# ThorLL/Element-Crush-Gym

Measured on AMD Instinct MI355X. Metric: env-steps/sec (batched boards) at 1/2/4/8 MI355X, 9×9×6; bit-exact vs CPU, higher is better.
Workload: dtype int8; 1 GPU; C3: 1,048,576 boards per GPU, 9x9x6, Match3Env.step x 7466 (step kernel + overflow fixup + autoreset; N>1: RCCL reward/done all-gather once after the last step); boards_per_gpu=1048576, num_moves=20, env_goal=500, parallelism=dp1, hw_queues=8, autoreset=True

## Files before the change

element-crush-gym_amd/csrc/m3_rules.hpp:

```cpp
#pragma once

#include <type_traits>

#include "m3_bitboard.hpp"
#include "m3_rng.hpp"

namespace m3 {

enum : int { PH_LOAD, PH_SWAP, PH_MATCH, PH_CLEAR, PH_DROP, PH_REFILL, PH_LEGAL, PH_NEXT, PH_RESET, PH_QUEUE,
             PH_STORE, PH_TBYTES, PH_TLOAD, PH_TATOM, PH_N };
template <class S, class = void>
struct HasProf : std::false_type {};
template <class S>
struct HasProf<S, std::void_t<decltype(S::PROF)>> : std::true_type {};
template <int K, class S>
M3_HD void mark(S& st) {
    if constexpr (HasProf<S>::value) st.template mark<K>();
}

constexpr int ceil_log2(int v) {
    int b = 0;
    while ((1 << b) < v) ++b;
    return b;
}

enum : uint32_t {
    FLAG_TERMINAL = 0x01u,
    FLAG_BAD_ACTION = 0x02u,
    FLAG_SHUFFLE_CAP = 0x04u,
    FLAG_NO_LEGAL = 0x08u,
    FLAG_SHUFFLED = 0x10u,
    FLAG_RNG_OVERFLOW = 0x20u,
    FLAG_GROUP_OVERFLOW = 0x40u,
    FLAG_RECOMPUTE = FLAG_RNG_OVERFLOW | FLAG_GROUP_OVERFLOW,
    FLAG_CASCADE_CAP = 0x100u,
    FLAG_RESET_CAP = 0x200u,
};
constexpr int CASCADE_CAP = 1 << 16;
template <class R, class = void>
struct DrawBounded : std::false_type {};
template <class R>
struct DrawBounded<R, std::void_t<decltype(R::DRAW_BOUNDED)>> : std::bool_constant<R::DRAW_BOUNDED> {};

template <class CF>
struct StaticDim;
template <class CF>
struct FrameDim;

template <int R_, int C_, int T_>
struct Cfg {
    static constexpr bool DYN = false;
    static constexpr int R = R_, C = C_, T = T_;
    static constexpr int N = R * C;
    static constexpr int W = (N + 31) / 32;
    static constexpr int BITS = ceil_log2(T + 1);
    static constexpr int TM = (1 << BITS) - 1;
    static constexpr int STM = (1 << (BITS + 1)) + 1 + TM;
    static constexpr int H = TM + 1;
    static constexpr int V = 2 * H;
    static constexpr int B = STM;
    static constexpr int M = TM + STM + 1;
    static constexpr int A = R * (C - 1) * 2;
    static constexpr int AW = (A + 31) / 32;
    static constexpr int NP = 7;
    static constexpr int MAXG = N / 3 + 1;
    static constexpr int SHUFFLE_CAP = 1024;
    static constexpr uint32_t TILE_RNG = (uint32_t)(T - 1);
    static constexpr uint32_t TILE_MASK = (1u << ceil_log2(T)) - 1u;
    static_assert(R >= 4 && C >= 4 && R <= 16 && C <= 16, "board size");
    static_assert(T >= 2 && BITS <= 4, "tile types must fit 4 bits");
    using Bd = BB<W>;
    using G = Geo<R, C, W>;
    using Dim = StaticDim<Cfg>;
};

template <int BITS_, int FS_ = 16>
struct FCfg {
    static constexpr bool DYN = true;
    static constexpr int FS = FS_;
    static_assert(FS == 16 || FS == 32, "frame side");
    static constexpr int R = FS, C = FS;
    static constexpr int N = R * C;
    static constexpr int W = N / 32;
    static constexpr int BITS = BITS_;
    static constexpr int TM = (1 << BITS) - 1;
    static constexpr int STM = (1 << (BITS + 1)) + 1 + TM;
    static constexpr int H = TM + 1;
    static constexpr int V = 2 * H;
    static constexpr int B = STM;
    static constexpr int M = TM + STM + 1;
    static constexpr int A = R * (C - 1) * 2;
    static constexpr int AW = (A + 31) / 32;
    static constexpr int NP = BITS >= 5 ? 8 : 7;
    static constexpr int MAXG = N / 3 + 1;
    static constexpr int SHUFFLE_CAP = 1024;
    static_assert(BITS >= 2 && BITS <= 5, "types 2..31");
    using Bd = BB<W>;
    using G = Geo<R, C, W>;
    using Dim = FrameDim<FCfg>;
};

constexpr int bits_for_types(int t) { return ceil_log2(t + 1); }

constexpr int MAX_FRAME = 32;
struct Shape {
    int rows, cols, types;
    int fs;
    uint32_t hreach[MAX_FRAME * MAX_FRAME / 32], vreach[MAX_FRAME * MAX_FRAME / 32];
};

M3_HD constexpr int frame_side(int rows, int cols) { return (rows > 16 || cols > 16) ? 32 : 16; }

M3_HD void decode_action(int action, int cols, int& r, int& c, bool& vertical) {
    const int AR = 2 * cols - 1, BR = cols - 1;
    if (action % AR >= BR) {
        c = action % AR - BR;
        r = (action - 3 - c) / AR;
        vertical = true;
    } else {
        c = action % AR;
        r = (action - c) / AR;
        vertical = false;
    }
}

M3_HD Shape make_shape(int rows, int cols, int types) {
    Shape s;
    s.rows = rows;
    s.cols = cols;
    s.types = types;
    s.fs = frame_side(rows, cols);
    for (int i = 0; i < MAX_FRAME * MAX_FRAME / 32; ++i) s.hreach[i] = s.vreach[i] = 0u;
    const int A = rows * (cols - 1) * 2;
    for (int a = 0; a < A; ++a) {
        int r, c;
        bool v;
        decode_action(a, cols, r, c, v);
        const int x = r * s.fs + c;
        if (r < 0 || x < 0 || x >= s.fs * s.fs) continue;
        (v ? s.vreach : s.hreach)[x >> 5] |= 1u << (x & 31);
    }
    return s;
}

template <class CF>
struct StaticDim {
    M3_HD constexpr StaticDim() {}
    M3_HD constexpr StaticDim(const Shape&) {}
    M3_HD static constexpr int rows() { return CF::R; }
    M3_HD static constexpr int cols() { return CF::C; }
    M3_HD static constexpr int cells() { return CF::N; }
    M3_HD static constexpr int actions() { return CF::A; }
    M3_HD static constexpr int aw() { return CF::AW; }
    M3_HD static constexpr uint32_t tile_rng() { return CF::TILE_RNG; }
    M3_HD static constexpr uint32_t tile_mask() { return CF::TILE_MASK; }
    M3_HD static constexpr typename CF::Bd valid() { return CF::G::valid(); }
};

M3_HD uint32_t in_vgpr(uint32_t x) {
#ifdef __HIP_DEVICE_COMPILE__
    uint32_t r;
    asm volatile("v_mov_b32 %0, %1" : "=v"(r) : "v"(x));
    return r;
#else
    return x;
#endif
}

template <class CF>
struct FrameDim {
    using Bd = typename CF::Bd;
    int r, c, a;
    uint32_t trng, tmask;
    Bd vmask;
    Bd hl, vl;
    M3_HD FrameDim(const Shape& s) : r(s.rows), c(s.cols), a(s.rows * (s.cols - 1) * 2) {
        trng = (uint32_t)(s.types - 1);
        uint32_t m = trng;
        m |= m >> 1; m |= m >> 2; m |= m >> 4;
        tmask = m;
        const uint32_t row = low_bits(c);
#pragma unroll
        for (int i = 0; i < CF::W; ++i) {
            if constexpr (CF::FS == 16) {
                const int r0 = 2 * i, r1 = 2 * i + 1;
                vmask.w[i] = (r0 < r ? row : 0u) | (r1 < r ? row << 16 : 0u);
            } else {
                vmask.w[i] = i < r ? row : 0u;
            }
            hl.w[i] = in_vgpr(s.hreach[i]);
            vl.w[i] = in_vgpr(s.vreach[i]);
            vmask.w[i] = in_vgpr(vmask.w[i]);
        }
    }
    M3_HD int rows() const { return r; }
    M3_HD int cols() const { return c; }
    M3_HD int cells() const { return r * c; }
    M3_HD int actions() const { return a; }
    M3_HD int aw() const { return (a + 31) / 32; }
    M3_HD uint32_t tile_rng() const { return trng; }
    M3_HD uint32_t tile_mask() const { return tmask; }
    M3_HD Bd valid() const { return vmask; }
};

M3_HD bool wave_any(bool p) {
#ifdef __HIP_DEVICE_COMPILE__
    return __any((int)p) != 0;
#elif defined(M3_HOST_WAVE_ANY)
    return M3_HOST_WAVE_ANY(p);
#else
    return p;
#endif
}

#ifndef M3_LEGAL_SLICED_W
#define M3_LEGAL_SLICED_W 5
#endif

template <class CF>
M3_HD typename CF::Bd tb_nonzero(const typename CF::Bd* P) {
    typename CF::Bd r = P[0];
#pragma unroll
    for (int p = 1; p < CF::BITS; ++p) r |= P[p];
    return r;
}

template <class CF, int NPU>
M3_HD typename CF::Bd special_mask(const typename CF::Bd* P) {
    typename CF::Bd r = P[CF::BITS];
#pragma unroll
    for (int p = CF::BITS + 1; p < NPU; ++p) r |= P[p];
    return r;
}

template <class CF, int D>
M3_HD typename CF::Bd tb_ne(const typename CF::Bd* P) {
    typename CF::Bd r = P[0] ^ at<D>(P[0]);
#pragma unroll
    for (int p = 1; p < CF::BITS; ++p) r |= P[p] ^ at<D>(P[p]);
    return r;
}
template <class CF, int D>
M3_HD typename CF::Bd tb_eq(const typename CF::Bd* P) {
    return ~tb_ne<CF, D>(P);
}

template <class CF, int NPU>
M3_HD int cell_value(const typename CF::Bd* P, int x) {
    const typename CF::Bd bm = CF::Bd::bit_at(x);
    int v = 0;
#pragma unroll
    for (int p = 0; p < NPU; ++p) v |= (int)((P[p] & bm).any()) << p;
    return v;
}

template <class CF, int NPU>
M3_HD void set_cell(typename CF::Bd* P, int x, int v) {
    const typename CF::Bd bm = CF::Bd::bit_at(x);
#pragma unroll
    for (int p = 0; p < NPU; ++p) {
        const uint32_t on = 0u - (uint32_t)((v >> p) & 1);
#pragma unroll
        for (int i = 0; i < CF::W; ++i) P[p].w[i] = (P[p].w[i] & ~bm.w[i]) | (bm.w[i] & on);
    }
}

template <int POS, int LEN, int W>
M3_HD uint32_t extract_bits(const BB<W>& b) {
    constexpr int q = POS >> 5, s = POS & 31;
    uint32_t lo = b.w[q] >> s;
    if constexpr (s != 0 && q + 1 < W) lo |= b.w[q + 1] << (32 - s);
    return LEN >= 32 ? lo : (lo & ((1u << (LEN & 31)) - 1u));
}

template <int K, int W>
M3_HD uint32_t wget(const BB<W>& a) {
    if constexpr (K >= 0 && K < W) return a.w[K];
    else return 0u;
}
template <int D, int I, int W>
M3_HD uint32_t wat(const BB<W>& a) {
    if constexpr (D == 0) {
        return wget<I>(a);
    } else if constexpr (D > 0) {
        constexpr int q = D / 32, s = D % 32;
        if constexpr (s == 0) return wget<I + q>(a);
        else return (wget<I + q>(a) >> s) | (wget<I + q + 1>(a) << (32 - s));
    } else {
        constexpr int q = (-D) / 32, s = (-D) % 32;
        if constexpr (s == 0) return wget<I - q>(a);
        else return (wget<I - q>(a) << s) | (wget<I - q - 1>(a) >> (32 - s));
    }
}
template <class CF, int A, int B, int I>
M3_HD uint32_t weq(const typename CF::Bd* P) {
    uint32_t r = 0u;
#pragma unroll
    for (int p = 0; p < CF::BITS; ++p) r |= wat<A, I>(P[p]) ^ wat<B, I>(P[p]);
    return ~r;
}
template <class CF, int I>
M3_HD void legal_word(const typename CF::Bd* P, const typename CF::Bd& z0, const typename CF::Bd& spec,
                      typename CF::Bd& HL, typename CF::Bd& VL) {
    using G = typename CF::G;
    constexpr int C = CF::C, R = CF::R;
    constexpr uint32_t RGE1 = G::row_ge(1).w[I], RGE2 = G::row_ge(2).w[I];
    constexpr uint32_t RLE2 = G::row_le(R - 2).w[I], RLE3 = G::row_le(R - 3).w[I], RLE4 = G::row_le(R - 4).w[I];
    constexpr uint32_t CGE1 = G::col_ge(1).w[I], CGE2 = G::col_ge(2).w[I];
    constexpr uint32_t CLE2 = G::col_le(C - 2).w[I], CLE3 = G::col_le(C - 3).w[I], CLE4 = G::col_le(C - 4).w[I];
    {
        const uint32_t spc = z0.w[I] | wat<1, I>(z0) | (spec.w[I] & wat<1, I>(spec));
        const uint32_t condA = CGE2 & weq<CF, -2, 1, I>(P) & weq<CF, -1, 1, I>(P);
        const uint32_t condB = CLE4 & weq<CF, 0, 2, I>(P) & weq<CF, 0, 3, I>(P);
        const uint32_t up = RGE1 & weq<CF, -C, 1, I>(P), dn = RLE2 & weq<CF, 1, C, I>(P);
        const uint32_t up2 = RGE2 & weq<CF, -2 * C, 1, I>(P), dn2 = RLE3 & weq<CF, 1, 2 * C, I>(P);
        const uint32_t ab1 = (up & dn) | (up & ~dn & up2) | (dn & ~up & dn2);
        const uint32_t upb = RGE1 & weq<CF, 1 - C, 0, I>(P), dnb = RLE2 & weq<CF, 0, C + 1, I>(P);
        const uint32_t up2b = RGE2 & weq<CF, 1 - 2 * C, 0, I>(P), dn2b = RLE3 & weq<CF, 0, 2 * C + 1, I>(P);
        const uint32_t ab2 = (upb & dnb) | (upb & ~dnb & up2b) | (dnb & ~upb & dn2b);
        HL.w[I] = CLE2 & (spc | ((condA | condB | ab1 | ab2) & ~weq<CF, 0, 1, I>(P)));
    }
    {
        const uint32_t spc = z0.w[I] | wat<C, I>(z0) | (spec.w[I] & wat<C, I>(spec));
        const uint32_t condA = RLE4 & weq<CF, 0, 2 * C, I>(P) & weq<CF, 0, 3 * C, I>(P);
        const uint32_t condB = RGE2 & weq<CF, -2 * C, C, I>(P) & weq<CF, -C, C, I>(P);
        const uint32_t l1 = CGE1 & weq<CF, 0, C - 1, I>(P), r1 = CLE2 & weq<CF, 0, C + 1, I>(P);
        const uint32_t l2 = CGE2 & weq<CF, 0, C - 2, I>(P), r2 = CLE3 & weq<CF, 0, C + 2, I>(P);
        const uint32_t lr1 = (l1 & r1) | (l1 & ~r1 & l2) | (r1 & ~l1 & r2);
        const uint32_t l1b = CGE1 & weq<CF, -1, C, I>(P), r1b = CLE2 & weq<CF, 1, C, I>(P);
        const uint32_t l2b = CGE2 & weq<CF, -2, C, I>(P), r2b = CLE3 & weq<CF, 2, C, I>(P);
        const uint32_t lr2 = (l1b & r1b) | (l1b & ~r1b & l2b) | (r1b & ~l1b & r2b);
        VL.w[I] = RLE2 & (spc | ((condA | condB | lr1 | lr2) & ~weq<CF, 0, C, I>(P)));
    }
}
template <class CF, int I = 0>
M3_HD void legal_words(const typename CF::Bd* P, const typename CF::Bd& z0, const typename CF::Bd& spec,
                       typename CF::Bd& HL, typename CF::Bd& VL) {
    if constexpr (I < CF::W) {
        legal_word<CF, I>(P, z0, spec, HL, VL);
        legal_words<CF, I + 1>(P, z0, spec, HL, VL);
    }
}

template <class CF>
M3_HD void legal_masks_all(const typename CF::Bd* P, const typename CF::Bd& spec,
                           typename CF::Bd& HL, typename CF::Bd& VL) {
    using Bd = typename CF::Bd;
    using G = typename CF::G;
    constexpr int C = CF::C, R = CF::R;
    constexpr Bd VALID = G::valid();
    const Bd z0 = VALID.andnot(tb_nonzero<CF>(P));
    if constexpr (M3_LEGAL_SLICED_W > 0 && CF::W >= M3_LEGAL_SLICED_W) {
        legal_words<CF>(P, z0, spec, HL, VL);
        return;
    }

    const Bd e1 = tb_eq<CF, 1>(P), e2 = tb_eq<CF, 2>(P), e3 = tb_eq<CF, 3>(P);
    const Bd ecm1 = tb_eq<CF, C - 1>(P), ecp1 = tb_eq<CF, C + 1>(P);
    const Bd e2cm1 = tb_eq<CF, 2 * C - 1>(P), e2cp1 = tb_eq<CF, 2 * C + 1>(P);
    const Bd ec = tb_eq<CF, C>(P), e2c = tb_eq<CF, 2 * C>(P), e3c = tb_eq<CF, 3 * C>(P);
    const Bd ecm2 = tb_eq<CF, C - 2>(P), ecp2 = tb_eq<CF, C + 2>(P);

    constexpr Bd RGE1 = G::row_ge(1), RGE2 = G::row_ge(2), RLE2 = G::row_le(R - 2), RLE3 = G::row_le(R - 3);
    constexpr Bd CGE1 = G::col_ge(1), CGE2 = G::col_ge(2), CLE2 = G::col_le(C - 2), CLE3 = G::col_le(C - 3);

    {
        const Bd spc = z0 | at<1>(z0) | (spec & at<1>(spec));
        const Bd condA = G::col_ge(2) & at<-2>(e3) & at<-1>(e2);
        const Bd condB = G::col_le(C - 4) & e2 & e3;
        const Bd up = RGE1 & at<-C>(ecp1), dn = RLE2 & at<1>(ecm1);
        const Bd up2 = RGE2 & at<-2 * C>(e2cp1), dn2 = RLE3 & at<1>(e2cm1);
        const Bd ab1 = (up & dn) | (up.andnot(dn) & up2) | (dn.andnot(up) & dn2);
        const Bd upb = RGE1 & at<1 - C>(ecm1), dnb = RLE2 & ecp1;
        const Bd up2b = RGE2 & at<1 - 2 * C>(e2cm1), dn2b = RLE3 & e2cp1;
        const Bd ab2 = (upb & dnb) | (upb.andnot(dnb) & up2b) | (dnb.andnot(upb) & dn2b);
        HL = CLE2 & (spc | ((condA | condB | ab1 | ab2).andnot(e1)));
    }
    {
        const Bd spc = z0 | at<C>(z0) | (spec & at<C>(spec));
        const Bd condA = G::row_le(R - 4) & e2c & e3c;
        const Bd condB = RGE2 & at<-2 * C>(e3c) & at<-C>(e2c);
        const Bd l1 = CGE1 & ecm1, r1 = CLE2 & ecp1, l2 = CGE2 & ecm2, r2 = CLE3 & ecp2;
        const Bd lr1 = (l1 & r1) | (l1.andnot(r1) & l2) | (r1.andnot(l1) & r2);
        const Bd l1b = CGE1 & at<-1>(ecp1), r1b = CLE2 & at<1>(ecm1);
        const Bd l2b = CGE2 & at<-2>(ecp2), r2b = CLE3 & at<2>(ecm2);
        const Bd lr2 = (l1b & r1b) | (l1b.andnot(r1b) & l2b) | (r1b.andnot(l1b) & r2b);
        VL = RLE2 & (spc | ((condA | condB | lr1 | lr2).andnot(ec)));
    }
}

template <class CF>
M3_HD void legal_masks(const typename CF::Bd* P, const typename CF::Bd& spec, typename CF::Bd& HL,
                       typename CF::Bd& VL, const typename CF::Dim& dm = typename CF::Dim{}) {
    legal_masks_all<CF>(P, spec, HL, VL);
    if constexpr (CF::DYN) {
        HL &= dm.hl;
        VL &= dm.vl;
    }
}

template <class CF, int ROW = 0>
M3_HD void action_bits_rows(const typename CF::Bd& HL, const typename CF::Bd& VL, uint32_t* act) {
    if constexpr (ROW < CF::R) {
        constexpr int C = CF::C;
        constexpr int POS = ROW * (2 * C - 1);
        const uint32_t h = extract_bits<ROW * C, C - 1>(HL);
        const uint32_t v = extract_bits<ROW * C, C>(VL);
        const uint32_t f = h | (v << (C - 1));
        constexpr int q = POS >> 5, s = POS & 31;
        act[q] |= f << s;
        if constexpr (s != 0 && s + 2 * C - 1 > 32 && q + 1 < CF::AW) act[q + 1] |= f >> (32 - s);
        action_bits_rows<CF, ROW + 1>(HL, VL, act);
    }
}
template <class CF>
M3_HD void action_bits_frame(const typename CF::Bd& HL, const typename CF::Bd& VL, uint32_t* act,
                             const typename CF::Dim& dm) {
    const int C = dm.cols(), L = 2 * C - 1, A = dm.actions();
    const uint64_t hm = ((uint64_t)1 << (C - 1)) - 1u, vm = ((uint64_t)1 << C) - 1u;
    auto row = [&](const typename CF::Bd& b, int r) -> uint64_t {
        if constexpr (CF::FS == 16) return (b.word_at(r >> 1) >> ((r & 1) * 16)) & 0xFFFFu;
        else return b.word_at(r);
    };
#pragma unroll
    for (int i = 0; i < CF::AW; ++i) act[i] = 0u;
    for (int r = 0; r < dm.rows(); ++r) {
        const int rv = C == 3 ? (r > 0 ? r - 1 : 0) : r;
        const uint64_t f = (row(HL, r) & hm) | ((row(VL, rv) & vm) << (C - 1));
        const int pos = r * L, q = pos >> 5, sh = pos & 31;
        const uint64_t lo = f << sh;
        const uint32_t w0 = (uint32_t)lo, w1 = (uint32_t)(lo >> 32), w2 = sh ? (uint32_t)(f >> (64 - sh)) : 0u;
#pragma unroll
        for (int i = 0; i < CF::AW; ++i)
            act[i] |= (i == q ? w0 : 0u) | (i == q + 1 ? w1 : 0u) | (i == q + 2 ? w2 : 0u);
    }
#pragma unroll
    for (int i = 0; i < CF::AW; ++i) {
        const int lim = A - 32 * i;
        act[i] = lim >= 32 ? act[i] : (lim <= 0 ? 0u : (act[i] & ((1u << lim) - 1u)));
    }
}

template <class CF>
M3_HD void action_bits(const typename CF::Bd& HL, const typename CF::Bd& VL, uint32_t* act,
                       const typename CF::Dim& dm = typename CF::Dim{}) {
    if constexpr (CF::DYN) {
        action_bits_frame<CF>(HL, VL, act, dm);
    } else {
#pragma unroll
        for (int i = 0; i < CF::AW; ++i) act[i] = 0u;
        action_bits_rows<CF, 0>(HL, VL, act);
    }
}


template <class CF, class RNG>
M3_HD int random_action(const uint32_t* act, RNG& rng) {
    int cnt = 0;
#pragma unroll
    for (int i = 0; i < CF::AW; ++i) cnt += __builtin_popcount(act[i]);
    if (cnt == 0) return -1;
    int k = (int)rand_masked(rng, (uint32_t)(cnt - 1));
    int res = 0;
    bool found = false;
#pragma unroll
    for (int i = 0; i < CF::AW; ++i) {
        const int c = __builtin_popcount(act[i]);
        if (!found) {
            if (k < c) {
                res = i * 32 + select_bit(act[i], k);
                found = true;
            } else {
                k -= c;
            }
        }
    }
    return res;
}

template <class CF>
struct ArrayStore {
    static constexpr int CAP = CF::MAXG;
    typename CF::Bd h[CAP];
    typename CF::Bd v[CAP];
    M3_HD typename CF::Bd get_h(int g) const { return h[g]; }
    M3_HD typename CF::Bd get_v(int g) const { return v[g]; }
    M3_HD bool put(int g, const typename CF::Bd& hh, const typename CF::Bd& vv) {
        h[g] = hh;
        v[g] = vv;
        return true;
    }
};

template <class CF, int CAP_>
struct SmallStore {
    static constexpr int CAP = CAP_;
    typename CF::Bd h[CAP];
    typename CF::Bd v[CAP];
    M3_HD typename CF::Bd get_h(int g) const { return h[g]; }
    M3_HD typename CF::Bd get_v(int g) const { return v[g]; }
    M3_HD bool put(int g, const typename CF::Bd& hh, const typename CF::Bd& vv) {
        h[g] = hh;
        v[g] = vv;
        return true;
    }
};

enum : int { MATCH_NONE = 0, MATCH_FOUND = 1, MATCH_OVERFLOW = -1 };

template <class CF>
M3_HD int multiset_select(const typename CF::Bd& hg, const typename CF::Bd& vg, int k) {
#pragma unroll
    for (int i = 0; i < CF::W; ++i) {
        const int c = __builtin_popcount(hg.w[i]) + __builtin_popcount(vg.w[i]);
        if (k < c) {
            uint32_t u = hg.w[i] | vg.w[i];
            while (u) {
                const int b = __builtin_ctz(u);
                const int m = (int)((hg.w[i] >> b) & 1u) + (int)((vg.w[i] >> b) & 1u);
                if (k < m) return i * 32 + b;
                k -= m;
                u &= u - 1u;
            }
        }
        k -= c;
    }
    return 0;
}

struct NoStore {
    static constexpr int CAP = 0;
};

template <class CF, bool SPAWN, class Store>
M3_HD int match_scan(const typename CF::Bd* P, typename CF::Bd& mask, typename CF::Bd* sw, Store& st) {
    using Bd = typename CF::Bd;
    using G = typename CF::G;
    constexpr int C = CF::C, R = CF::R;
    constexpr Bd CLE2 = G::col_le(C - 2), RLE2 = G::row_le(R - 2);

    const Bd nz = tb_nonzero<CF>(P);
    const Bd e1h = CLE2 & tb_eq<CF, 1>(P);
    const Bd e1v = RLE2 & tb_eq<CF, C>(P);
    const Bd h3 = nz & e1h & at<1>(e1h);
    const Bd v3 = nz & e1v & at<C>(e1v);
    Bd cand = h3 | v3;
    mask = Bd::zero();
    if constexpr (SPAWN) {
        sw[0] = Bd::zero();
        sw[1] = Bd::zero();
        sw[2] = Bd::zero();
    }
    if (!cand.any()) return MATCH_NONE;

    const Bd dh2 = e1h & at<1>(e1h), dh4 = dh2 & at<2>(dh2), dh8 = dh4 & at<4>(dh4);
    const Bd dv2 = e1v & at<C>(e1v), dv4 = dv2 & at<2 * C>(dv2), dv8 = dv4 & at<4 * C>(dv4);
    Bd dh16, dv16;
    if constexpr (C > 16) dh16 = dh8 & at<8>(dh8);
    if constexpr (R > 16) dv16 = dv8 & at<8 * C>(dv8);

    int ng = 0;
    Bd vruns = Bd::zero();
    while (cand.any()) {
        const int x = cand.lowest();
        const Bd bx = Bd::bit_at(x);
        Bd rh = Bd::zero(), rv = Bd::zero();
        if ((h3 & bx).any()) {
            rh = bx;
            rh |= at<-1>(rh & e1h);
            rh |= at<-2>(rh & dh2);
            rh |= at<-4>(rh & dh4);
            if constexpr (C > 8) rh |= at<-8>(rh & dh8);
            if constexpr (C > 16) rh |= at<-16>(rh & dh16);
        }
        if ((v3 & bx).any()) {
            rv = bx;
            rv |= at<-C>(rv & e1v);
            rv |= at<-2 * C>(rv & dv2);
            rv |= at<-4 * C>(rv & dv4);
            if constexpr (R > 8) rv |= at<-8 * C>(rv & dv8);
            if constexpr (R > 16) rv |= at<-16 * C>(rv & dv16);
        }
        const Bd run = rh | rv;
        mask |= run;
        cand = cand.andnot(run | bx);
        if constexpr (SPAWN) {
            int g = -1;
            if ((rh & vruns).any()) {
                for (int gi = 0; gi < ng; ++gi) {
                    if ((st.get_v(gi) & rh).any()) { g = gi; break; }
                }
            }
            if (g < 0) {
                if (ng == Store::CAP || !st.put(ng, rh, rv)) return MATCH_OVERFLOW;
                ++ng;
            } else if (!st.put(g, st.get_h(g) | rh, st.get_v(g) | rv)) {
                return MATCH_OVERFLOW;
            }
            vruns |= rv;
        }
    }
    if constexpr (SPAWN) {
        for (int gi = 0; gi < ng; ++gi) {
            const Bd hg = st.get_h(gi), vg = st.get_v(gi);
            const int len = hg.popc() + vg.popc();
            if (len <= 3) continue;
            int centre, kind;
            if (!vg.any()) {
                centre = hg.lowest() + len / 2;
                kind = len > 4 ? 4 : 2;
            } else if (!hg.any()) {
                centre = vg.lowest() + (len / 2) * C;
                kind = len > 4 ? 4 : 1;
            } else {
                centre = multiset_select<CF>(hg, vg, len / 2);
                kind = 3;
            }
            const Bd bm = Bd::bit_at(centre);
            sw[0] = sw[0].andnot(bm);
            sw[1] = sw[1].andnot(bm);
            sw[2] = sw[2].andnot(bm);
            if (kind & 1) sw[0] |= bm;
            if (kind & 2) sw[1] |= bm;
            if (kind & 4) sw[2] |= bm;
        }
    }
    return MATCH_FOUND;
}

#ifndef M3_FAST_MATCH
#define M3_FAST_MATCH 1
#endif
template <class CF, class Store>
M3_HD int get_matches(const typename CF::Bd* P, typename CF::Bd& mask, typename CF::Bd* sw, Store& st) {
    if constexpr (M3_FAST_MATCH) {
        using Bd = typename CF::Bd;
        using G = typename CF::G;
        constexpr int C = CF::C, R = CF::R;
        constexpr Bd CLE2 = G::col_le(C - 2), RLE2 = G::row_le(R - 2);
        const Bd nz = tb_nonzero<CF>(P);
        const Bd e1h = CLE2 & tb_eq<CF, 1>(P);
        const Bd e1v = RLE2 & tb_eq<CF, C>(P);
        const Bd h3 = nz & e1h & at<1>(e1h);
        const Bd v3 = nz & e1v & at<C>(e1v);
        if (!(h3 | v3).any()) {
            mask = Bd::zero();
            sw[0] = sw[1] = sw[2] = Bd::zero();
            return MATCH_NONE;
        }
        const Bd hc = h3 | at<-1>(h3) | at<-2>(h3);
        const Bd vc = v3 | at<-C>(v3) | at<-2 * C>(v3);
        const Bd h4 = h3 & at<1>(h3), v4 = v3 & at<C>(v3);
        const bool six = (h4 & at<2>(h4)).any() || (v4 & at<2 * C>(v4)).any();
        if (!(hc & vc).any() && !six) {
            const Bd hf = h4.andnot(at<-1>(e1h));
            const Bd vf = v4.andnot(at<-C>(e1v));
            const Bd hf5 = hf & at<2>(h3), vf5 = vf & at<2 * C>(v3);
            mask = hc | vc;
            sw[0] = at<-2 * C>(vf.andnot(vf5));
            sw[1] = at<-2>(hf.andnot(hf5));
            sw[2] = at<-2>(hf5) | at<-2 * C>(vf5);
            return MATCH_FOUND;
        }
    }
    return match_scan<CF, true>(P, mask, sw, st);
}

template <class CF>
M3_HD bool get_match_mask_scan(const typename CF::Bd* P, typename CF::Bd& mask) {
    NoStore ns;
    return match_scan<CF, false>(P, mask, nullptr, ns) != MATCH_NONE;
}

template <class CF>
M3_HD bool get_match_mask(const typename CF::Bd* P, typename CF::Bd& mask) {
    using Bd = typename CF::Bd;
    using G = typename CF::G;
    constexpr int C = CF::C, R = CF::R;
    constexpr Bd CLE2 = G::col_le(C - 2), RLE2 = G::row_le(R - 2);
    const Bd nz = tb_nonzero<CF>(P);
    const Bd e1h = CLE2 & tb_eq<CF, 1>(P);
    const Bd e1v = RLE2 & tb_eq<CF, C>(P);
    const Bd h3 = nz & e1h & at<1>(e1h);
    const Bd v3 = nz & e1v & at<C>(e1v);
    if (!(h3 | v3).any()) {
        mask = Bd::zero();
        return false;
    }
    const Bd hc = h3 | at<-1>(h3) | at<-2>(h3);
    const Bd vc = v3 | at<-C>(v3) | at<-2 * C>(v3);
    const Bd hin = hc.andnot(h3.andnot(at<-1>(h3)));
    const Bd vin = vc.andnot(v3.andnot(at<-C>(v3)));
    if (!((h3 & vin) | (v3 & hin)).any()) {
        mask = hc | vc;
        return true;
    }
    return get_match_mask_scan<CF>(P, mask);
}

M3_HD void py_slice(int start, int stop, int n, int& lo, int& hi) {
    if (start < 0) {
        start += n;
        if (start < 0) start = 0;
    }
    if (start > n) start = n;
    if (stop > n) stop = n;
    lo = start;
    hi = stop > start ? stop : start;
}

template <class CF, int NPU>
M3_HD typename CF::Bd fire_specials(const typename CF::Bd* P, typename CF::Bd z,
                                   const typename CF::Dim& dm = typename CF::Dim{}) {
    using Bd = typename CF::Bd;
    using G = typename CF::G;
    constexpr int BITS = CF::BITS, C = CF::C;
    const int R = dm.rows(), CB = dm.cols();
    const Bd spz = z & special_mask<CF, NPU>(P);
    const Bd kh = P[BITS].andnot(P[BITS + 1]);
    const Bd kv = P[BITS + 1].andnot(P[BITS]);
    const Bd kb = P[BITS] & P[BITS + 1];
    Bd trig = spz & (kh | kv | kb);
    Bd add = Bd::zero();
    while (trig.any()) {
        const int x = trig.lowest();
        trig.pop_lowest();
        const int i = x / C, j = x % C;
        if (kh.test(x)) {
            add |= G::row_band(i, i + 1);
        } else if (kv.test(x)) {
            add |= G::col_band(j, j + 1);
        } else {
            int rl, rh, cl, ch;
            py_slice(j - 1, j + 1, R, rl, rh);
            py_slice(i - 1, i + 1, CB, cl, ch);
            add |= G::row_band(rl, rh) & G::col_band(cl, ch);
        }
    }
    if constexpr (CF::DYN) return (z | add) & dm.valid();
    return z | add;
}

template <class CF, int NPU>
M3_HD int score(const typename CF::Bd* P, const typename CF::Bd& z) {
    using Bd = typename CF::Bd;
    constexpr int BITS = CF::BITS;
    const Bd spec = special_mask<CF, NPU>(P);
    Bd hi2 = P[BITS + 2];
#pragma unroll
    for (int p = BITS + 3; p < NPU; ++p) hi2 |= P[p];
    Bd other = P[0];
#pragma unroll
    for (int p = 1; p < NPU; ++p)
        if (p != BITS + 2) other |= P[p];
    const Bd eqm = P[BITS + 2].andnot(other);
    const Bd kb = P[BITS] & P[BITS + 1];
    const Bd lt = spec.andnot(hi2 | kb);
    const Bd zs = z & spec;
    const int n_all = z.popc(), n_spec = zs.popc();
    const int n_m = (z & eqm).popc(), n_lt = (z & lt).popc();
    return 2 * (n_all - n_spec) + 250 * n_m + 25 * n_lt + 50 * (n_spec - n_m - n_lt);
}

template <class CF, int NPU>
M3_HD void merge_clip(typename CF::Bd* P, const typename CF::Bd& z, const typename CF::Bd* sw) {
    using Bd = typename CF::Bd;
    constexpr int BITS = CF::BITS;
#pragma unroll
    for (int p = 0; p < NPU; ++p) P[p] = P[p].andnot(z);
    P[BITS] |= sw[0];
    P[BITS + 1] |= sw[1];
    P[BITS + 2] |= sw[2];
    Bd low = P[0];
#pragma unroll
    for (int p = 1; p < 5; ++p) low |= P[p];
    Bd hi = P[6];
#pragma unroll
    for (int p = 7; p < CF::NP; ++p) hi |= P[p];
    const Bd cl = (P[5] & low) | hi;
#pragma unroll
    for (int p = 0; p < 5; ++p) P[p] = P[p].andnot(cl);
    P[5] |= cl;
#pragma unroll
    for (int p = 6; p < CF::NP; ++p) P[p] = Bd::zero();
}

template <class CF>
M3_HD typename CF::Bd gravity_decomp(typename CF::Bd* P, const typename CF::Dim& dm = typename CF::Dim{}) {
    using Bd = typename CF::Bd;
    constexpr int C = CF::C, R = CF::R, NPU = 6;
    constexpr int STAGES = ceil_log2(R);
    const Bd VALID = dm.valid();
    Bd m = P[0];
#pragma unroll
    for (int p = 1; p < NPU; ++p) m |= P[p];
    Bd mk = at<C>(VALID.andnot(m));
    auto stage = [&](auto S) {
        constexpr int D = (1 << decltype(S)::value) * C;
        Bd mp = mk ^ at<C>(mk);
        if constexpr (R > 3) mp ^= at<2 * C>(mp);
        if constexpr (R > 5) mp ^= at<4 * C>(mp);
        if constexpr (R > 9) mp ^= at<8 * C>(mp);
        if constexpr (R > 17) mp ^= at<16 * C>(mp);
        const Bd mv = mp & m;
        if (wave_any(mv.any())) {
            m = m.andnot(mv) | at<-D>(mv);
#pragma unroll
            for (int p = 0; p < NPU; ++p) {
                const Bd t = P[p] & mv;
                P[p] = P[p].andnot(mv) | at<-D>(t);
            }
        }
        mk = mk.andnot(mp);
    };
    stage(std::integral_constant<int, 0>{});
    if constexpr (STAGES > 1) if (wave_any(mk.any())) {
        stage(std::integral_constant<int, 1>{});
        if constexpr (STAGES > 2) if (wave_any(mk.any())) {
            stage(std::integral_constant<int, 2>{});
            if constexpr (STAGES > 3) if (wave_any(mk.any())) {
                stage(std::integral_constant<int, 3>{});
                if constexpr (STAGES > 4) if (wave_any(mk.any())) stage(std::integral_constant<int, 4>{});
            }
        }
    }
    return VALID.andnot(m);
}

template <class CF>
M3_HD typename CF::Bd gravity(typename CF::Bd* P, const typename CF::Dim& dm = typename CF::Dim{}) {
    return gravity_decomp<CF>(P, dm);
}

template <class CF, class RNG>
M3_HD void refill(typename CF::Bd* P, const typename CF::Bd& em, RNG& rng,
                  const typename CF::Dim& dm = typename CF::Dim{}) {
    using Bd = typename CF::Bd;
    constexpr int C = CF::C, R = CF::R;
    if (!em.any()) return;
    uint32_t tops = em.w[0] & low_bits(C);
    int c = __builtin_ctz(tops);
    int r = 0;
    const uint32_t tmask = dm.tile_mask(), trng = dm.tile_rng();
    for (;;) {
        uint32_t v = rng.next32() & tmask;
        if (rng.overflow) break;
        if (v > trng) continue;
        v += 1u;
        const int x = r * C + c;
        const Bd bm = Bd::bit_at(x);
#pragma unroll
        for (int p = 0; p < CF::BITS; ++p) {
            const uint32_t on = 0u - ((v >> p) & 1u);
#pragma unroll
            for (int i = 0; i < CF::W; ++i) P[p].w[i] |= bm.w[i] & on;
        }
        if (r + 1 < R && em.test(x + C)) {
            ++r;
        } else {
            tops &= ~(1u << c);
            if (!tops) break;
            c = __builtin_ctz(tops);
            r = 0;
        }
    }
}

template <class CF, class RNG>
M3_HD void shuffle_rows(typename CF::Bd* P, RNG& rng, const typename CF::Dim& dm = typename CF::Dim{}) {
    using Bd = typename CF::Bd;
    constexpr int C = CF::C, R = CF::R, NPU = 6;
    rng.reseed();
    const Bd sp = special_mask<CF, NPU>(P);
    if constexpr (R > 16) {
        static_assert(C == 32, "one row per word");
        uint8_t perm[R];
#pragma unroll
        for (int i = 0; i < R; ++i) perm[i] = (uint8_t)i;
        for (int i = dm.rows() - 1; i >= 1; --i) {
            const int j = (int)rand_masked(rng, (uint32_t)i);
            const uint8_t a = perm[i];
            perm[i] = perm[j];
            perm[j] = a;
        }
        Bd out[NPU];
#pragma unroll
        for (int i = 0; i < R; ++i) {
            const int src = perm[i];
#pragma unroll
            for (int p = 0; p < NPU; ++p) out[p].w[i] = P[p].word_at(src);
        }
#pragma unroll
        for (int p = 0; p < NPU; ++p) P[p] = out[p].andnot(sp) | (P[p] & sp);
        return;
    }
    uint64_t idx = 0;
#pragma unroll
    for (int i = 0; i < R; ++i) idx |= (uint64_t)i << (4 * i);
    for (int i = dm.rows() - 1; i >= 1; --i) {
        const int j = (int)rand_masked(rng, (uint32_t)i);
        const uint64_t a = (idx >> (4 * i)) & 0xFull, b = (idx >> (4 * j)) & 0xFull;
        idx &= ~((0xFull << (4 * i)) | (0xFull << (4 * j)));
        idx |= (b << (4 * i)) | (a << (4 * j));
    }
    Bd out[NPU];
#pragma unroll
    for (int p = 0; p < NPU; ++p) out[p] = Bd::zero();
#pragma unroll
    for (int i = 0; i < R; ++i) {
        const int src = (int)((idx >> (4 * i)) & 0xFull);
        const int sb = src * C;
        const int q = sb >> 5, s = sb & 31;
#pragma unroll
        for (int p = 0; p < NPU; ++p) {
            const uint32_t lo = P[p].word_at(q), hi = P[p].word_at(q + 1);
            uint32_t f = s ? ((lo >> s) | (hi << ((32 - s) & 31))) : lo;
            f &= low_bits(C);
            const int dpos = i * C;
            const int dq = dpos >> 5, ds = dpos & 31;
            out[p].w[dq] |= f << ds;
            if (ds + C > 32 && dq + 1 < CF::W) out[p].w[dq + 1] |= f >> (32 - ds);
        }
    }
#pragma unroll
    for (int p = 0; p < NPU; ++p) P[p] = out[p].andnot(sp) | (P[p] & sp);
}

template <class CF, class RNG, class Store>
M3_HD bool apply_begin(typename CF::Bd* P, int n_actions, int action, RNG& rng, uint32_t& flags,
                       typename CF::Bd& HL, typename CF::Bd& VL, Store& st, int& reward,
                       const typename CF::Dim& dm = typename CF::Dim{}) {
    using Bd = typename CF::Bd;
    using G = typename CF::G;
    constexpr int C = CF::C, TM = CF::TM;
    constexpr int H = CF::H, V = CF::V, B = CF::B, M = CF::M;
    const int R = dm.rows(), CB = dm.cols();
    const Bd VALID = dm.valid();
    flags = 0u;
    reward = 0;
    mark<PH_LOAD>(st);
    if (n_actions < 1 || action < 0 || action >= dm.actions()) {
        flags = (n_actions < 1) ? FLAG_TERMINAL : FLAG_BAD_ACTION;
        legal_masks<CF>(P, special_mask<CF, CF::NP>(P), HL, VL, dm);
        return false;
    }
    rng.reseed();
    const int AR = 2 * CB - 1, BR = CB - 1;
    int sr, sc, tr, tc;
    if (action % AR >= BR) {
        sc = action % AR - BR;
        sr = (action - 3 - sc) / AR;
        tr = sr + 1;
        tc = sc;
    } else {
        sc = action % AR;
        sr = (action - sc) / AR;
        tr = sr;
        tc = sc + 1;
    }
    const int s = sr * C + sc, t = tr * C + tc;
    const int tok1 = cell_value<CF, CF::NP>(P, s), tok2 = cell_value<CF, CF::NP>(P, t);
    {
        const Bd st = Bd::bit_at(s) | Bd::bit_at(t);
        const int d = tok1 ^ tok2;
#pragma unroll
        for (int p = 0; p < CF::NP; ++p)
            if ((d >> p) & 1) P[p] ^= st;
    }
    const int ty1 = tok2 > TM ? tok2 : 0, ty2 = tok1 > TM ? tok1 : 0;
    auto are = [&](int a, int b) { return (ty1 == a && ty2 == b) || (ty2 == a && ty1 == b); };

    Bd sw[3] = {Bd::zero(), Bd::zero(), Bd::zero()};
    Bd zr;
    if (are(M, M)) {
        zr = VALID;
    } else if (are(M, B) || are(M, H) || are(M, V) || are(M, 0)) {
        zr = Bd::zero();
    } else if (are(B, B)) {
        const int r0 = tr - 2 < 0 ? 0 : tr - 2, r1 = tr + 2 > R ? R : tr + 2;
        const int c0 = tc - 2 < 0 ? 0 : tc - 2, c1 = tc + 2 > CB ? CB : tc + 2;
        zr = G::row_band(r0, r1) & G::col_band(c0, c1);
    } else if (are(B, H) || are(B, V)) {
        const int r0 = tr - 2 < 0 ? 0 : tr - 2, r1 = tr + 2 > R ? R : tr + 2;
        const int c0 = tc - 2 < 0 ? 0 : tc - 2, c1 = tc + 2 > CB ? CB : tc + 2;
        zr = G::col_band(c0, c1) | G::row_band(r0, r1);
    } else if (are(H, V)) {
        zr = G::row_band(0, tc < R ? tc : R) | G::row_band(tr, R);
    } else {
        mark<PH_SWAP>(st);
        if (get_matches<CF>(P, zr, sw, st) == MATCH_OVERFLOW) {
            flags |= FLAG_GROUP_OVERFLOW;
            return false;
        }
        mark<PH_MATCH>(st);
    }
    mark<PH_SWAP>(st);
    Bd z = zr | VALID.andnot(tb_nonzero<CF>(P));
    z = fire_specials<CF, CF::NP>(P, z, dm);
    reward += score<CF, CF::NP>(P, z);
    merge_clip<CF, CF::NP>(P, z, sw);
    mark<PH_CLEAR>(st);
    return true;
}

enum : int { CAS_PAUSED = 0, CAS_DONE = 1, CAS_SETTLED = 2, CAS_DEAD = 3 };
enum : int { CASX_STOP_SETTLED = 1, CASX_STOP_DEAD = 2 };

template <class CF, int OPTS, class RNG, class Store>
M3_HD int apply_cascade_ex(typename CF::Bd* P, RNG& rng, uint32_t& flags, typename CF::Bd& HL,
                           typename CF::Bd& VL, Store& st, int& reward, int limit, bool start_settled,
                           const typename CF::Dim& dm = typename CF::Dim{}) {
    using Bd = typename CF::Bd;
    const Bd VALID = dm.valid();
    Bd sw[3];
    int it = 0;
    bool settled = start_settled;
    for (;;) {
        Bd mask;
        bool found = false;
        if (!settled) {
            if constexpr (CF::DYN) {
                int xr = -1;
                bool live = true;
                for (;;) {
                    if (!wave_any(live)) break;
                    if (!live) continue;
                    if (it == limit) {
                        xr = CAS_PAUSED;
                        live = false;
                        continue;
                    }
                    if constexpr (CF::DYN || !DrawBounded<RNG>::value) {
                        if (it >= CASCADE_CAP) {
                            flags |= FLAG_CASCADE_CAP;
                            live = false;
                            continue;
                        }
                    }
                    ++it;
                    const Bd em = gravity<CF>(P, dm);
                    mark<PH_DROP>(st);
                    refill<CF>(P, em, rng, dm);
                    mark<PH_REFILL>(st);
                    if (rng.overflow) {
                        live = false;
                        continue;
                    }
                    const int mr = get_matches<CF>(P, mask, sw, st);
                    mark<PH_MATCH>(st);
                    if (mr == MATCH_OVERFLOW) {
                        flags |= FLAG_GROUP_OVERFLOW;
                        xr = CAS_DONE;
                        live = false;
                        continue;
                    }
                    if (mr != MATCH_FOUND) {
                        live = false;
                        continue;
                    }
                    Bd z = mask | VALID.andnot(tb_nonzero<CF>(P));
                    z = fire_specials<CF, 6>(P, z, dm);
                    reward += score<CF, 6>(P, z);
                    merge_clip<CF, 6>(P, z, sw);
                    mark<PH_CLEAR>(st);
                }
                if (xr >= 0) return xr;
            } else {
            for (;;) {
                if (it == limit) return CAS_PAUSED;
                if constexpr (CF::DYN || !DrawBounded<RNG>::value) {
                    if (it >= CASCADE_CAP) {
                        flags |= FLAG_CASCADE_CAP;
                        break;
                    }
                }
                ++it;
                const Bd em = gravity<CF>(P, dm);
                mark<PH_DROP>(st);
                refill<CF>(P, em, rng, dm);
                mark<PH_REFILL>(st);
                if (rng.overflow) break;
                const int mr = get_matches<CF>(P, mask, sw, st);
                mark<PH_MATCH>(st);
                if (mr == MATCH_OVERFLOW) {
                    flags |= FLAG_GROUP_OVERFLOW;
                    return CAS_DONE;
                }
                if (mr != MATCH_FOUND) break;
                Bd z = mask | VALID.andnot(tb_nonzero<CF>(P));
                z = fire_specials<CF, 6>(P, z, dm);
                reward += score<CF, 6>(P, z);
                merge_clip<CF, 6>(P, z, sw);
                mark<PH_CLEAR>(st);
            }
            }
            if (rng.overflow) break;
            if constexpr ((OPTS & CASX_STOP_SETTLED) != 0) return CAS_SETTLED;
        }
        settled = false;
        legal_masks<CF>(P, special_mask<CF, 6>(P), HL, VL, dm);
        mark<PH_LEGAL>(st);
        if (HL.any() || VL.any()) break;
        if constexpr ((OPTS & CASX_STOP_DEAD) != 0) return CAS_DEAD;
        int shuffles = 0;
        while (!found && !(HL.any() || VL.any())) {
            if (shuffles >= CF::SHUFFLE_CAP) {
                flags |= FLAG_SHUFFLE_CAP;
                break;
            }
            shuffle_rows<CF>(P, rng, dm);
            flags |= FLAG_SHUFFLED;
            ++shuffles;
            const int mr = get_matches<CF>(P, mask, sw, st);
            if (mr == MATCH_OVERFLOW) {
                flags |= FLAG_GROUP_OVERFLOW;
                return CAS_DONE;
            }
            found = mr == MATCH_FOUND;
            if (!found) legal_masks<CF>(P, special_mask<CF, 6>(P), HL, VL, dm);
        }
        if (!found) break;
        Bd z = mask | VALID.andnot(tb_nonzero<CF>(P));
        z = fire_specials<CF, 6>(P, z, dm);
        reward += score<CF, 6>(P, z);
        merge_clip<CF, 6>(P, z, sw);
        mark<PH_CLEAR>(st);
    }
    if (rng.overflow) flags |= FLAG_RNG_OVERFLOW;
    return CAS_DONE;
}

template <class CF, class RNG, class Store>
M3_HD bool apply_cascade(typename CF::Bd* P, RNG& rng, uint32_t& flags, typename CF::Bd& HL,
                         typename CF::Bd& VL, Store& st, int& reward, int limit,
                         const typename CF::Dim& dm = typename CF::Dim{}) {
    return apply_cascade_ex<CF, 0>(P, rng, flags, HL, VL, st, reward, limit, false, dm) != CAS_PAUSED;
}

template <class CF, class RNG>
struct Cont {
    static_assert(std::is_trivially_copyable<RNG>::value && sizeof(RNG) % 4 == 0, "RNG state must be words");
    static constexpr int PW = 6 * CF::W;
    static constexpr int RW = (int)(sizeof(RNG) / 4);
    static constexpr int WORDS = PW + RW + 2;
    template <class Put>
    static M3_HD void save(const typename CF::Bd* P, const RNG& rng, int reward, uint32_t flags, Put put) {
#pragma unroll
        for (int p = 0; p < 6; ++p)
#pragma unroll
            for (int i = 0; i < CF::W; ++i) put(p * CF::W + i, P[p].w[i]);
        uint32_t r[RW];
        __builtin_memcpy(r, &rng, sizeof(RNG));
#pragma unroll
        for (int i = 0; i < RW; ++i) put(PW + i, r[i]);
        put(PW + RW, (uint32_t)reward);
        put(PW + RW + 1, flags);
    }
    template <class Get>
    static M3_HD void load(typename CF::Bd* P, RNG& rng, int& reward, uint32_t& flags, Get get) {
#pragma unroll
        for (int p = 0; p < 6; ++p)
#pragma unroll
            for (int i = 0; i < CF::W; ++i) P[p].w[i] = get(p * CF::W + i);
#pragma unroll
        for (int p = 6; p < CF::NP; ++p) P[p] = CF::Bd::zero();
        uint32_t r[RW];
#pragma unroll
        for (int i = 0; i < RW; ++i) r[i] = get(PW + i);
        __builtin_memcpy(&rng, r, sizeof(RNG));
        reward = (int)get(PW + RW);
        flags = get(PW + RW + 1);
    }
};

template <class CF, class RNG, class Store>
M3_HD int apply_action(typename CF::Bd* P, int n_actions, int action, RNG& rng, uint32_t& flags,
                       typename CF::Bd& HL, typename CF::Bd& VL, Store& st,
                       const typename CF::Dim& dm = typename CF::Dim{}) {
    int reward;
    if (apply_begin<CF>(P, n_actions, action, rng, flags, HL, VL, st, reward, dm))
        apply_cascade<CF>(P, rng, flags, HL, VL, st, reward, -1, dm);
    return (flags & FLAG_RECOMPUTE) ? 0 : reward;
}

template <class CF, class RNG, class S>
M3_HD void init_board(typename CF::Bd* P, RNG& mt, S& st, const typename CF::Dim& dm = typename CF::Dim{}) {
    using Bd = typename CF::Bd;
#pragma unroll
    for (int p = 0; p < CF::NP; ++p) P[p] = Bd::zero();
    const int RB = dm.rows(), CB = dm.cols();
    const uint32_t tmask = dm.tile_mask(), trng = dm.tile_rng();
    auto fill = [&](const Bd* only) {
        int r = 0, c = 0;
        while (r < RB) {
            uint32_t v = mt.next32() & tmask;
            if (mt.overflow) return;
            if (v > trng) continue;
            v += 1u;
            const int x = r * CF::C + c;
            if (!only || only->test(x)) set_cell<CF, CF::BITS>(P, x, (int)v);
            if (++c == CB) {
                c = 0;
                ++r;
            }
        }
    };
    mark<PH_LOAD>(st);
    fill(nullptr);
    mark<PH_REFILL>(st);
    Bd mask;
    for (;;) {
        if (mt.overflow) break;
        const bool any = get_match_mask<CF>(P, mask);
        mark<PH_MATCH>(st);
        if (!any) break;
        fill(&mask);
        mark<PH_REFILL>(st);
    }
}


template <class CF>
struct TileGen {
#ifndef M3_TW9
#define M3_TW9 10
#endif
    static constexpr int TWMAX = CF::N <= 128 ? M3_TW9 : 32;
    static constexpr int MAXR = 624 / CF::N + 2;
    static_assert(TWMAX > CF::W + 1, "a round's read window fits the ring");
    static M3_HD uint32_t slot(uint32_t q) {
        if constexpr ((TWMAX & (TWMAX - 1)) == 0) return q & (uint32_t)(TWMAX - 1);
        else return q % (uint32_t)TWMAX;
    }
};


template <class CF, class RNG, class RawSink, class AccSink, class S = NoStore>
M3_HD bool init_board_tiles(typename CF::Bd* P, RNG& g, uint32_t* tm, uint32_t* pos, int stride, uint32_t& draws,
                            uint32_t rawn, RawSink raw_sink, AccSink acc_sink, S* ps = nullptr,
                            uint32_t kcap = 624u) {
    using Bd = typename CF::Bd;
    using G = typename CF::G;
    constexpr int TW = TileGen<CF>::TWMAX, N = CF::N, MAXR = TileGen<CF>::MAXR;
    constexpr Bd VALID = G::valid();
    static_assert(!CF::DYN, "frame boards reset on FullMT (k_init_fix_lane)");
    static_assert(CF::TILE_RNG > 0u, "randint(1, 2) consumes no draws");
    uint32_t cur[CF::BITS];
#pragma unroll
    for (int p = 0; p < CF::BITS; ++p) cur[p] = 0u;
    uint32_t nt = 0u, accw = 0u;
    uint32_t floor_tile = 0u;
    bool ring_full = false;
    constexpr uint32_t RING_TILES = 32u * (uint32_t)(TW - CF::W - 1);
    auto gen_to = [&](uint32_t kend) {
        for (uint32_t k = g.k; k < kend; ++k) {
            const uint32_t v = g.next32();
            const uint32_t t = v & CF::TILE_MASK;
            const bool ok = t <= CF::TILE_RNG;
            if (k < rawn) {
                raw_sink(k, v);
                accw |= (uint32_t)ok << (k & 31u);
                if ((k & 31u) == 31u) {
                    acc_sink(k >> 5, accw);
                    accw = 0u;
                }
            }
            if (ok && nt - floor_tile >= RING_TILES) ring_full = true;
            if (ok && !ring_full) {
                const uint32_t val = t + 1u, sh = nt & 31u;
#pragma unroll
                for (int p = 0; p < CF::BITS; ++p) cur[p] |= ((val >> p) & 1u) << sh;
                ++nt;
                if ((nt & 31u) == 0u) {
#pragma unroll
                    for (int p = 0; p < CF::BITS; ++p) {
                        tm[(p * TW + (int)TileGen<CF>::slot((nt >> 5) - 1u)) * stride] = cur[p];
                        cur[p] = 0u;
                    }
                }
                if (nt % (uint32_t)N == 0u && nt / (uint32_t)N < (uint32_t)MAXR) pos[(nt / N) * stride] = k + 1u;
            }
        }
#pragma unroll
        for (int p = 0; p < CF::BITS; ++p)
            tm[(p * TW + (int)TileGen<CF>::slot(nt >> 5)) * stride] = cur[p];
    };
    auto ensure = [&](uint32_t need, bool want) {
        while (wave_any(want && !ring_full && nt < need) && g.k < kcap) {
            const uint32_t kend = g.k + 64u < kcap ? g.k + 64u : kcap;
            gen_to(kend);
        }
        return !want || nt >= need;
    };
    auto take = [&](uint32_t j, Bd* T) {
        const uint32_t q = j >> 5;
        const uint32_t sh = j & 31u;
#pragma unroll
        for (int p = 0; p < CF::BITS; ++p) {
            uint32_t lo = tm[(p * TW + (int)TileGen<CF>::slot(q)) * stride];
#pragma unroll
            for (int i = 0; i < CF::W; ++i) {
                const uint32_t hi = tm[(p * TW + (int)TileGen<CF>::slot(q + (uint32_t)i + 1u)) * stride];
                T[p].w[i] = sh ? ((lo >> sh) | (hi << (32u - sh))) : lo;
                lo = hi;
            }
            T[p] &= VALID;
        }
    };
    if constexpr (HasProf<S>::value) ps->template mark<PH_LOAD>();
#pragma unroll
    for (int p = 0; p < CF::NP; ++p) P[p] = Bd::zero();
    bool ok = ensure((uint32_t)N, true);
    if (ok) take(0u, P);
    floor_tile = (uint32_t)N;
    if constexpr (HasProf<S>::value) ps->template mark<PH_REFILL>();
    uint32_t rounds = 1u;
    bool live = ok;
    Bd mask;
    for (;;) {
        const bool any = live && get_match_mask<CF>(P, mask);
        if constexpr (HasProf<S>::value) ps->template mark<PH_MATCH>();
        live = any;
        const uint32_t need = (rounds + 1u) * (uint32_t)N;
        const bool have = ensure(need, live);
        if (live && !have) ok = false;
        live = live && have;
        if (!wave_any(live)) break;
        if (live) {
            Bd T[CF::BITS];
            take(rounds * (uint32_t)N, T);
#pragma unroll
            for (int p = 0; p < CF::BITS; ++p) P[p] = P[p].andnot(mask) | (T[p] & mask);
            ++rounds;
            floor_tile = rounds * (uint32_t)N;
        } else {
            floor_tile = nt;
        }
        if constexpr (HasProf<S>::value) ps->template mark<PH_REFILL>();
    }
    draws = ok ? pos[rounds * stride] : 0u;
    if (g.k < rawn) gen_to(rawn);
    if (rawn & 31u) acc_sink(rawn >> 5, accw);
    if constexpr (HasProf<S>::value) ps->template mark<PH_NEXT>();
    return ok;
}

M3_HD void transpose8(uint32_t& lo, uint32_t& hi) {
    uint32_t t;
    t = (lo ^ (lo >> 7)) & 0x00AA00AAu; lo ^= t ^ (t << 7);
    t = (hi ^ (hi >> 7)) & 0x00AA00AAu; hi ^= t ^ (t << 7);
    t = (lo ^ (lo >> 14)) & 0x0000CCCCu; lo ^= t ^ (t << 14);
    t = (hi ^ (hi >> 14)) & 0x0000CCCCu; hi ^= t ^ (t << 14);
    t = (lo ^ (hi << 4)) & 0xF0F0F0F0u; lo ^= t; hi ^= t >> 4;
}

template <class CF>
M3_HD void planes_from_words(const uint32_t* cw, typename CF::Bd* P) {
    constexpr int NW = (CF::N + 3) / 4;
#pragma unroll
    for (int p = 0; p < CF::NP; ++p) P[p] = CF::Bd::zero();
#pragma unroll
    for (int g = 0; g < (CF::N + 7) / 8; ++g) {
        uint32_t lo = (2 * g < NW) ? cw[2 * g] : 0u;
        uint32_t hi = (2 * g + 1 < NW) ? cw[2 * g + 1] : 0u;
        transpose8(lo, hi);
        const int q = (8 * g) >> 5, sh = (8 * g) & 31;
#pragma unroll
        for (int p = 0; p < CF::NP; ++p) {
            const uint32_t byte = ((p < 4 ? lo : hi) >> (8 * (p & 3))) & 0xFFu;
            P[p].w[q] |= byte << sh;
        }
    }
    constexpr typename CF::Bd VALID = CF::G::valid();
#pragma unroll
    for (int p = 0; p < CF::NP; ++p) P[p] &= VALID;
}

template <class CF>
M3_HD void words_from_planes(const typename CF::Bd* P, uint32_t* cw) {
    constexpr int NW = (CF::N + 3) / 4;
#pragma unroll
    for (int g = 0; g < (CF::N + 7) / 8; ++g) {
        const int q = (8 * g) >> 5, sh = (8 * g) & 31;
        uint32_t lo = 0u, hi = 0u;
#pragma unroll
        for (int p = 0; p < CF::NP; ++p) {
            const uint32_t byte = (P[p].w[q] >> sh) & 0xFFu;
            if (p < 4) lo |= byte << (8 * p);
            else hi |= byte << (8 * (p - 4));
        }
        transpose8(lo, hi);
        if (2 * g < NW) cw[2 * g] = lo;
        if (2 * g + 1 < NW) cw[2 * g + 1] = hi;
    }
}


template <class CF>
M3_HD uint32_t frame_row(const typename CF::Bd& b, int r) {
    if constexpr (CF::FS == 16) return (b.w[r >> 1] >> ((r & 1) * 16)) & 0xFFFFu;
    else return b.w[r];
}
template <class CF>
M3_HD void frame_row_merge(typename CF::Bd& b, int r, uint32_t v, uint32_t m) {
    if constexpr (CF::FS == 16) {
        const int sh = (r & 1) * 16;
        b.w[r >> 1] = (b.w[r >> 1] & ~(m << sh)) | ((v & m) << sh);
    } else {
        b.w[r] = (b.w[r] & ~m) | (v & m);
    }
}

template <class CF>
M3_HD void frame_from_bytes(const uint8_t* src, typename CF::Bd* P, const typename CF::Dim& dm) {
    static_assert(CF::DYN, "frame layout");
    constexpr int FS = CF::FS, NG = FS / 8;
    const int RB = dm.rows(), CB = dm.cols();
#pragma unroll
    for (int p = 0; p < CF::NP; ++p) P[p] = CF::Bd::zero();
#pragma unroll
    for (int r = 0; r < CF::R; ++r) {
        if (r < RB) {
            const uint8_t* row = src + r * CB;
            uint32_t w[2 * NG];
#pragma unroll
            for (int k = 0; k < 2 * NG; ++k) w[k] = 0u;
#pragma unroll
            for (int k = 0; k < FS; ++k)
                if (k < CB) w[k >> 2] |= (uint32_t)row[k] << (8 * (k & 3));
#pragma unroll
            for (int g = 0; g < NG; ++g) transpose8(w[2 * g], w[2 * g + 1]);
#pragma unroll
            for (int p = 0; p < CF::NP; ++p) {
                uint32_t v = 0u;
#pragma unroll
                for (int g = 0; g < NG; ++g) v |= ((w[2 * g + (p < 4 ? 0 : 1)] >> (8 * (p & 3))) & 0xFFu) << (8 * g);
                frame_row_merge<CF>(P[p], r, v, 0xFFFFFFFFu >> (32 - FS));
            }
        }
    }
}

template <class CF>
M3_HD void frame_to_bytes(const typename CF::Bd* P, uint8_t* dst, const typename CF::Dim& dm) {
    static_assert(CF::DYN, "frame layout");
    constexpr int FS = CF::FS, NG = FS / 8;
    const int RB = dm.rows(), CB = dm.cols();
#pragma unroll
    for (int r = 0; r < CF::R; ++r) {
        if (r < RB) {
            uint32_t w[2 * NG];
#pragma unroll
            for (int k = 0; k < 2 * NG; ++k) w[k] = 0u;
#pragma unroll
            for (int p = 0; p < CF::NP; ++p) {
                const uint32_t bits = frame_row<CF>(P[p], r);
#pragma unroll
                for (int g = 0; g < NG; ++g) w[2 * g + (p < 4 ? 0 : 1)] |= ((bits >> (8 * g)) & 0xFFu) << (8 * (p & 3));
            }
#pragma unroll
            for (int g = 0; g < NG; ++g) transpose8(w[2 * g], w[2 * g + 1]);
            uint8_t* row = dst + r * CB;
#pragma unroll
            for (int k = 0; k < FS; ++k)
                if (k < CB) row[k] = (uint8_t)(w[k >> 2] >> (8 * (k & 3)));
        }
    }
}

template <class CF, class RNG>
M3_HD void fill_round_frame(typename CF::Bd* P, RNG& mt, const typename CF::Bd* only, const typename CF::Dim& dm) {
    const int RB = dm.rows(), CB = dm.cols();
    const uint32_t tmask = dm.tile_mask(), trng = dm.tile_rng(), rowm = low_bits(CB);
#pragma unroll
    for (int r = 0; r < CF::R; ++r) {
        if (r < RB) {
            uint32_t t[CF::BITS];
#pragma unroll
            for (int p = 0; p < CF::BITS; ++p) t[p] = 0u;
            for (int c = 0; c < CB; ++c) {
                uint32_t v;
                do {
                    v = mt.next32() & tmask;
                } while (v > trng);
                v += 1u;
#pragma unroll
                for (int p = 0; p < CF::BITS; ++p) t[p] |= ((v >> p) & 1u) << c;
            }
            const uint32_t m = only ? frame_row<CF>(*only, r) & rowm : rowm;
#pragma unroll
            for (int p = 0; p < CF::BITS; ++p) frame_row_merge<CF>(P[p], r, t[p], m);
        }
    }
}

}
```

Baseline: 2.681 billion env-steps/s.

## Replace per-cell refill loop with batched RNG draw and bit-parallel column placement

For static 9x9 boards using the chained MT generator, refill now draws all needed tile values first into per-bitplane bitmasks, inlining the MT recurrence in a tight loop. It then scatters them into the board with bitfield extracts and 24-bit multiplies that place whole column runs at once. This replaces the per-cell loop, which built a one-bit mask and OR'd every bitplane word for each cell. If any lane in the wave needs more than 32 cells, the old loop still runs, and other configurations also keep the old path.

```diff
diff --git a/element-crush-gym_amd/csrc/m3_rules.hpp b/element-crush-gym_amd/csrc/m3_rules.hpp
--- a/element-crush-gym_amd/csrc/m3_rules.hpp
+++ b/element-crush-gym_amd/csrc/m3_rules.hpp
@@ -833,8 +833,8 @@
 }
 
 template <class CF, class RNG>
-M3_HD void refill(typename CF::Bd* P, const typename CF::Bd& em, RNG& rng,
-                  const typename CF::Dim& dm = typename CF::Dim{}) {
+M3_HD void refill_loop(typename CF::Bd* P, const typename CF::Bd& em, RNG& rng,
+                       const typename CF::Dim& dm = typename CF::Dim{}) {
     using Bd = typename CF::Bd;
     constexpr int C = CF::C, R = CF::R;
     if (!em.any()) return;
@@ -863,6 +863,112 @@
             c = __builtin_ctz(tops);
             r = 0;
         }
+    }
+}
+
+M3_HD uint32_t ubfe(uint32_t src, uint32_t off, uint32_t n) {
+#ifdef __HIP_DEVICE_COMPILE__
+    return __builtin_amdgcn_ubfe(src, off, n);
+#else
+    return (src >> (off & 31u)) & ((1u << (n & 31u)) - 1u);
+#endif
+}
+M3_HD uint32_t umul24(uint32_t a, uint32_t b) {
+#ifdef __HIP_DEVICE_COMPILE__
+    return __umul24(a, b);
+#else
+    return a * b;
+#endif
+}
+
+template <class RNG>
+struct IsChainMT : std::false_type {};
+template <uint32_t LIMIT>
+struct IsChainMT<ChainMTT<LIMIT>> : std::true_type {};
+
+template <class CF>
+M3_HD void refill_place(typename CF::Bd* P, const typename CF::Bd& em, const uint32_t* S) {
+    using G = typename CF::G;
+    constexpr int C = CF::C, R = CF::R, W = CF::W, NB = CF::BITS;
+    static_assert(R == 9 && C == 9 && W == 3, "the row groups below are laid out for 9 x 9");
+    constexpr uint32_t K = 0x010101u, M = 0x040201u;
+    const uint32_t need = (uint32_t)em.popc();
+    uint32_t g0[NB], g1[NB], g2[NB];
+#pragma unroll
+    for (int p = 0; p < NB; ++p) g0[p] = g1[p] = g2[p] = 0u;
+    uint32_t off = 0u;
+#pragma unroll
+    for (int c = 0; c < C; ++c) {
+        const uint32_t nxt = c + 1 < C ? (uint32_t)(em & G::col_le(c)).popc() : need;
+        const uint32_t h = nxt - off;
+#pragma unroll
+        for (int p = 0; p < NB; ++p) {
+            const uint32_t x = ubfe(S[p], off, h);
+            const uint32_t lo = x & 0x3Fu, hi = (x >> 6) & 7u;
+            const uint32_t m = c < 8 ? umul24(lo, K << c) : umul24(lo << c, K);
+            const uint32_t n = c < 8 ? umul24(hi, K << c) : umul24(hi << c, K);
+            g0[p] |= m & (M << c);
+            g1[p] |= m & (M << (c + 3));
+            g2[p] |= n & (M << c);
+        }
+        off = nxt;
+    }
+#pragma unroll
+    for (int p = 0; p < NB; ++p) {
+        P[p].w[0] |= g0[p] | (g1[p] << 24);
+        P[p].w[1] |= (g1[p] >> 8) | (g2[p] << 22);
+        P[p].w[2] |= g2[p] >> 10;
+    }
+}
+
+template <class CF, class RNG>
+M3_HD void refill(typename CF::Bd* P, const typename CF::Bd& em, RNG& rng,
+                  const typename CF::Dim& dm = typename CF::Dim{}) {
+    if constexpr (!CF::DYN && CF::N <= 128 && IsChainMT<RNG>::value) {
+        const uint32_t need = (uint32_t)em.popc();
+#if defined(M3_HOST_REFILL_HOOK) && !defined(__HIP_DEVICE_COMPILE__)
+        M3_HOST_REFILL_HOOK(need);
+#endif
+        if (wave_any(need > 32u)) {
+            refill_loop<CF>(P, em, rng, dm);
+            return;
+        }
+        constexpr uint32_t tmask = CF::TILE_MASK, trng = CF::TILE_RNG;
+        uint32_t S[CF::BITS];
+#pragma unroll
+        for (int p = 0; p < CF::BITS; ++p) S[p] = 0u;
+        uint32_t left = need, bit = 1u;
+        {
+            uint32_t a_lo = rng.a_lo, a_hi = rng.a_hi, k = rng.k;
+            while (left != 0u && k < 227u) {
+                const uint32_t lo1 = mt_init_next(a_lo, k + 1u);
+                const uint32_t v = mt_temper(a_hi ^ mt_twist(a_lo, lo1)) & tmask;
+                a_hi = mt_init_next(a_hi, k + 398u);
+                a_lo = lo1;
+                k += 1u;
+                const uint32_t acc = v <= trng ? 1u : 0u;
+                const uint32_t sel = acc ? bit : 0u;
+#pragma unroll
+                for (int p = 0; p < CF::BITS; ++p) S[p] |= (0u - (((v + 1u) >> p) & 1u)) & sel;
+                bit <<= acc;
+                left -= acc;
+            }
+            rng.a_lo = a_lo;
+            rng.a_hi = a_hi;
+            rng.k = k;
+        }
+        while (left != 0u) {
+            const uint32_t v = rng.next32() & tmask;
+            if (rng.overflow) break;
+            if (v > trng) continue;
+#pragma unroll
+            for (int p = 0; p < CF::BITS; ++p) S[p] |= (0u - (((v + 1u) >> p) & 1u)) & bit;
+            bit <<= 1;
+            left -= 1u;
+        }
+        refill_place<CF>(P, em, S);
+    } else {
+        refill_loop<CF>(P, em, rng, dm);
     }
 }
 
```

Result: faster. 2.818 billion env-steps/s (median of 6 runs) (+5.1%).
